# locuslab/icnn

Hardware: NVIDIA H100
Metric: inner-loop solves/sec (batch x iters) (higher is better)
Workload: dtype f32 (K1 PICNN f/grad) + f64 (K2 bundle solve)

## Files before the change

icnn_b200/csrc/bundle_pc.cu:

```cuda
#include "bundle_pc_kernel.cuh"

#include <cstdio>
#include <cstdlib>

namespace icnn {

#define ICNN_PC_DECL(NAME) cudaError_t launch_pc_##NAME(const PcArgs& a, const PcConfig& c, int B, cudaStream_t st)
ICNN_PC_DECL(1x1); ICNN_PC_DECL(1x2);
ICNN_PC_DECL(1x1_scalar); ICNN_PC_DECL(1x2_scalar);
ICNN_PC_DECL(8x2);
ICNN_PC_DECL(16x2); ICNN_PC_DECL(16x4);
ICNN_PC_DECL(v3_8x4);

ICNN_PC_DECL(1x1) { return launch_pc<1, 1, true>(a, c, B, st); }
ICNN_PC_DECL(1x2) { return launch_pc<1, 2, true>(a, c, B, st); }
ICNN_PC_DECL(1x1_scalar) { return launch_pc<1, 1, false>(a, c, B, st); }
ICNN_PC_DECL(1x2_scalar) { return launch_pc<1, 2, false>(a, c, B, st); }

struct PcTestEnv { bool v3, split5, seed, twolog; int pfa, pfb; };
static PcTestEnv pc_test_env() {
  PcTestEnv e = {true, false, true, false, 1, 8};
  if (const char* v = getenv("ICNN_PC_V3")) e.v3 = v[0] != '0';
  if (const char* v = getenv("ICNN_PC_LEGACY")) e.split5 = v[0] == '1';
  if (const char* v = getenv("ICNN_PC_SEED")) e.seed = v[0] != '0';
  if (const char* v = getenv("ICNN_PC_TWOLOG")) e.twolog = v[0] == '1';
  if (const char* v = getenv("ICNN_PC_PREFETCH")) {
    int pa = 0, pb = 0;
    if (sscanf(v, "%d,%d", &pa, &pb) == 2 && pa >= 0 && pa <= 8 && pb >= 0 && pb <= 64) { e.pfa = pa; e.pfb = pb; }
  }
  return e;
}

static bool pc_fits(int n, int KS, int wps, int nch, bool v3, PcConfig* out) {
  if (n > 128 * wps * nch) return false;
  PcConfig c;
  c.wps = wps; c.nch = nch; c.v3 = v3;
  c.npad = (n + 15) & ~15;
  c.vec = (n & 3) == 0;
  if (!c.vec && wps > 1) return false;
  c.smem = sizeof(double) * pc_group_doubles(c.npad, KS, wps, v3);
  if (c.smem > 227 * 1024) return false;
  if (v3) {
    if (!c.vec || 2 * (c.smem + 1024) > 228 * 1024) return false;
    c.minb = 2;
  } else if (wps == 16) c.minb = 1;
  else if (wps == 1) c.minb = 2;
  else
    c.minb = (c.smem + 1024) * (24 / wps) <= 228 * 1024 ? 3 : 2;
  *out = c;
  return true;
}

bool pick_pc(int n, int KS, PcConfig* out) {
  const bool allow_v3 = pc_test_env().v3;
  if (KS > 62) return false;
  if (n <= 128) return pc_fits(n, KS, 1, 1, false, out);
  if (n <= 256) return pc_fits(n, KS, 1, 2, false, out);
  if (n <= 1024) return false;
  if (n <= 2048) return pc_fits(n, KS, 8, 2, false, out);
  if (n <= 4096) return (allow_v3 && pc_fits(n, KS, 8, 4, true, out)) || pc_fits(n, KS, 16, 2, false, out);
  return pc_fits(n, KS, 16, 4, false, out);
}

int bundle_pc_launch(const icnn_bundle_cfg* cfg, const icnn_bundle_bufs* b, int t, const PcConfig& c, cudaStream_t st) {
  const PcTestEnv env = pc_test_env();
  PcArgs a;
  a.b = *b; a.c = *cfg; a.t = t; a.npad = c.npad;
  a.split5 = env.split5; a.seed = env.seed; a.twolog = env.twolog; a.pfa = env.pfa; a.pfb = env.pfb;
  cudaError_t e;
  if (c.v3) e = launch_pc_v3_8x4(a, c, b->B, st);
  else if (c.wps == 16) e = c.nch == 2 ? launch_pc_16x2(a, c, b->B, st) : launch_pc_16x4(a, c, b->B, st);
  else if (c.wps == 8) e = launch_pc_8x2(a, c, b->B, st);
  else if (c.vec) e = c.nch == 1 ? launch_pc_1x1(a, c, b->B, st) : launch_pc_1x2(a, c, b->B, st);
  else e = c.nch == 1 ? launch_pc_1x1_scalar(a, c, b->B, st) : launch_pc_1x2_scalar(a, c, b->B, st);
  if (e != cudaSuccess) {
    set_error("bundle_pc launch (wps=%d nch=%d v3=%d smem=%zu): %s", c.wps, c.nch, (int)c.v3, c.smem, cudaGetErrorString(e));
    return ICNN_E_CUDA;
  }
  return ICNN_OK;
}

}
```

icnn_b200/csrc/bundle_pc_kernel.cuh:

```cuda
#pragma once
#include "bundle_step_kernel.cuh"

namespace icnn {

struct PcArgs {
  icnn_bundle_bufs b;
  icnn_bundle_cfg c;
  int t;
  int npad;
  int pfa;
  int pfb;
  bool split5;
  bool seed;
  bool twolog;
#ifdef ICNN_PC_PHASES
  unsigned long long* ph;
#endif
};

enum PcPhase {
  PC_PH_APPEND = 0,
  PC_PH_SEED,
  PC_PH_U0,
  PC_PH_SWEEPA,
  PC_PH_KXK,
  PC_PH_SWEEPB,
  PC_PH_SIGMA,
  PC_PH_DIR2,
  PC_PH_UPDATE,
  PC_PH_COMMIT,
  PC_NPH
};
constexpr int PC_PH_SLOTS = 32;
#ifdef ICNN_PC_PHASES
#define PC_PHASE_START() long long pc_ph_t = clock64()
#define PC_PHASE(i)                                                                                              \
  do {                                                                                                           \
    if (threadIdx.x == 0) {                                                                                      \
      const long long pc_c = clock64();                                                                          \
      atomicAdd(A.ph + ((size_t)A.t * PC_NPH + (i)) * PC_PH_SLOTS + (blockIdx.x & (PC_PH_SLOTS - 1)),            \
                (unsigned long long)(pc_c - pc_ph_t));                                                           \
      pc_ph_t = pc_c;                                                                                            \
    }                                                                                                            \
  } while (0)
#else
#define PC_PHASE_START() do {} while (0)
#define PC_PHASE(i) do {} while (0)
#endif

__device__ __forceinline__ void prefetch_l2(const void* p) { asm volatile("prefetch.global.L2 [%0];" ::"l"(p)); }

constexpr int PC_NKV = 18;
constexpr int PC_NKV_V3 = 12;

__host__ __device__ inline size_t pc_group_doubles(int npad, int KS, int wps, bool v3) {
  size_t d = (size_t)(v3 ? 3 : 4) * npad + (size_t)KS * (KS + 1) / 2 +
             (size_t)(v3 ? PC_NKV_V3 : PC_NKV) * KS + KS  +
             8 * wps  + 16  + 4 ;
  return (d + 1) & ~(size_t)1;
}

__device__ __forceinline__ int lidx(int r, int c) { return r * (r + 1) / 2 + c; }

__device__ __forceinline__ double chol_dot(const double* a, const double* b, int c) {
  double t0 = 0.0, t1 = 0.0, t2 = 0.0, t3 = 0.0;
  int p = 0;
  for (; p + 3 < c; p += 4) {
    t0 = fma(a[p], b[p], t0);
    t1 = fma(a[p + 1], b[p + 1], t1);
    t2 = fma(a[p + 2], b[p + 2], t2);
    t3 = fma(a[p + 3], b[p + 3], t3);
  }
  for (; p < c; ++p) t0 = fma(a[p], b[p], t0);
  return (t0 + t1) + (t2 + t3);
}
template <bool K32>
__device__ __forceinline__ bool warp_cholesky_impl(double* L, double* invd, int k, int lane) {
  bool ok = true;
  const int r0 = lane, r1 = lane + 32;
  const int o0 = lidx(r0, 0), o1 = lidx(r1, 0);
  for (int c = 0; c < k; ++c) {
    const int oc = lidx(c, 0);
    double s0 = 0.0, s1 = 0.0;
    if (r0 >= c && r0 < k) s0 = L[o0 + c] - chol_dot(L + o0, L + oc, c);
    if (!K32) { if (r1 >= c && r1 < k) s1 = L[o1 + c] - chol_dot(L + o1, L + oc, c); }
    const double piv = K32 ? __shfl_sync(0xffffffffu, s0, c) : __shfl_sync(0xffffffffu, (c < 32) ? s0 : s1, c & 31);
    if (!(piv > 0.0) || !isfinite(piv)) { ok = false; break; }
    const double inv = rsqrt(piv);
    if (r0 > c && r0 < k) L[o0 + c] = s0 * inv;
    if (!K32) { if (r1 > c && r1 < k) L[o1 + c] = s1 * inv; }
    if (lane == 0) { L[oc + c] = piv * inv; invd[c] = inv; }
    __syncwarp();
  }
  __syncwarp();
  return ok;
}
__device__ inline bool warp_cholesky_p(double* L, double* invd, int k, int lane) {
  return k <= 32 ? warp_cholesky_impl<true>(L, invd, k, lane) : warp_cholesky_impl<false>(L, invd, k, lane);
}

template <int NR, bool K32>
__device__ __forceinline__ void warp_chol_fwd_impl(const double* L, const double* invd, int k, double (&b0)[NR],
                                                   double (&b1)[NR], int lane) {
  const int r0 = lane, r1 = lane + 32;
  const int o0 = lidx(r0, 0), o1 = lidx(r1, 0);
  for (int i = 0; i < k; ++i) {
    const double di = invd[i];
    const double l0 = (r0 > i && r0 < k) ? L[o0 + i] : 0.0;
    const double l1 = (!K32 && r1 > i && r1 < k) ? L[o1 + i] : 0.0;
#pragma unroll
    for (int q = 0; q < NR; ++q) {
      const double xi = (K32 ? __shfl_sync(0xffffffffu, b0[q], i) : __shfl_sync(0xffffffffu, (i < 32) ? b0[q] : b1[q], i & 31)) * di;
      b0[q] = (r0 == i) ? xi : fma(-l0, xi, b0[q]);
      if (!K32) b1[q] = (r1 == i) ? xi : fma(-l1, xi, b1[q]);
    }
  }
}
template <int NR, bool K32>
__device__ __forceinline__ void warp_chol_bwd_impl(const double* L, const double* invd, int k, double (&b0)[NR],
                                                   double (&b1)[NR], int lane) {
  const int r0 = lane, r1 = lane + 32;
  for (int i = k - 1; i >= 0; --i) {
    const double di = invd[i];
    const int oi = lidx(i, 0);
    const double l0 = (r0 < i) ? L[oi + r0] : 0.0;
    const double l1 = (!K32 && r1 < i) ? L[oi + r1] : 0.0;
#pragma unroll
    for (int q = 0; q < NR; ++q) {
      const double xi = (K32 ? __shfl_sync(0xffffffffu, b0[q], i) : __shfl_sync(0xffffffffu, (i < 32) ? b0[q] : b1[q], i & 31)) * di;
      b0[q] = (r0 == i) ? xi : fma(-l0, xi, b0[q]);
      if (!K32) b1[q] = (r1 == i) ? xi : fma(-l1, xi, b1[q]);
    }
  }
}
template <int NR, bool K32>
__device__ __forceinline__ void warp_chol_solve_impl(const double* L, const double* invd, int k, double (&b0)[NR],
                                                     double (&b1)[NR], int lane) {
  warp_chol_fwd_impl<NR, K32>(L, invd, k, b0, b1, lane);
  warp_chol_bwd_impl<NR, K32>(L, invd, k, b0, b1, lane);
}
template <int NR>
__device__ inline void warp_chol_solve_p(const double* L, const double* invd, int k, double (&b0)[NR],
                                         double (&b1)[NR], int lane) {
  if (k <= 32) warp_chol_solve_impl<NR, true>(L, invd, k, b0, b1, lane);
  else warp_chol_solve_impl<NR, false>(L, invd, k, b0, b1, lane);
}
template <bool K32>
__device__ __forceinline__ double warp_chol_solve_fwdsq_impl(const double* L, const double* invd, int k, double (&b0)[1],
                                                             double (&b1)[1], int lane) {
  warp_chol_fwd_impl<1, K32>(L, invd, k, b0, b1, lane);
  const double f0 = lane < k ? b0[0] : 0.0, f1 = (!K32 && lane + 32 < k) ? b1[0] : 0.0;
  const double fs = Grp<1>::wsum(fma(f0, f0, f1 * f1));
  warp_chol_bwd_impl<1, K32>(L, invd, k, b0, b1, lane);
  return fs;
}
__device__ inline double warp_chol_solve_fwdsq_p(const double* L, const double* invd, int k, double (&b0)[1],
                                                 double (&b1)[1], int lane) {
  return k <= 32 ? warp_chol_solve_fwdsq_impl<true>(L, invd, k, b0, b1, lane)
                 : warp_chol_solve_fwdsq_impl<false>(L, invd, k, b0, b1, lane);
}

__device__ __forceinline__ double step2(double v0, double d0, bool ok0, double v1, double d1, bool ok1) {
  double a = 1e300;
  bool any = false;
  if (ok0 && d0 < 0.0) { a = -v0 / d0; any = true; }
  if (ok1 && d1 < 0.0) { a = fmin(a, -v1 / d1); any = true; }
  a = Grp<1>::wmin(a);
  any = __any_sync(0xffffffffu, any);
  return any ? a : 1.0;
}

template <int WPS>
struct PcRed {
  double* red;
  int par;
  template <class G>
  __device__ __forceinline__ double sum(const G& g, double v) {
    v = Grp<WPS>::wsum(v);
    if (WPS == 1) { __syncwarp(); return v; }
    double* r = red + par * 4 * WPS;
    par ^= 1;
    if (g.lane == 0) r[g.warp] = v;
    g.sync();
    double a = 0.0;
#pragma unroll
    for (int w = 0; w < WPS; ++w) a += r[w];
    return a;
  }
  template <class G>
  __device__ __forceinline__ void min2(const G& g, double& a, double& b) {
    a = Grp<WPS>::wmin(a);
    b = Grp<WPS>::wmin(b);
    if (WPS == 1) { __syncwarp(); return; }
    double* r = red + par * 4 * WPS;
    par ^= 1;
    if (g.lane == 0) { r[g.warp] = a; r[WPS + g.warp] = b; }
    g.sync();
    double ra = r[0], rb = r[WPS];
#pragma unroll
    for (int w = 1; w < WPS; ++w) { ra = fmin(ra, r[w]); rb = fmin(rb, r[WPS + w]); }
    a = ra; b = rb;
  }
};

__device__ __forceinline__ double dweight(double y) { return fma(-y, y, y); }

template <int T, bool IL>
__device__ __forceinline__ int pc_tc(int cb, int npad) { return IL ? ::min(T, (npad - cb) >> 2) : 1; }
template <int T, bool IL>
__device__ __forceinline__ int pc_pos(int e, int npad) {
  if (!IL) return e;
  const int cb = e & ~(4 * T - 1);
  return cb + (e & 3) * pc_tc<T, IL>(cb, npad) + ((e - cb) >> 2);
}

template <int WPS, int NA, int NB, bool TRI, bool PSEUDO, bool VEC, bool IL, class G>
__device__ __forceinline__ void gram_sweep_pc(const G& g, const float* const* rowp, int k, int n, const double* yv,
                                              const double* rv, double* Lp, double* qk, double* wk, double* scratch,
                                              int scap, int a0, int b0, int pfd = 0) {
  constexpr int NT = TRI ? NA * (NA + 1) / 2 : NA * NB;
  constexpr int NL = TRI ? NB : NA + NB;
  double acc[NT][2];
#pragma unroll
  for (int t = 0; t < NT; ++t) acc[t][0] = acc[t][1] = 0.0;
  const int r = g.lane >> 2, q = g.lane & 3;
  const float* rp[NL];
  bool rok[NL];
#pragma unroll
  for (int b = 0; b < NL; ++b) {
    const int blk = TRI ? (b0 + b) : (b < NA ? a0 + b : b0 + (b - NA));
    const int row = blk * 8 + r - 2;
    rok[b] = row >= 0 && row < k;
    rp[b] = rowp[rok[b] ? row : 0] + 4 * q;
  }
  const bool ps = PSEUDO && r < 2;
  const double* yq = yv + 4 * q;
  const double* rq = rv + 4 * q;
  const int ngrp = (n + 15) >> 4;
  constexpr int NG = (NT <= 6) ? 2 : 1;
#pragma unroll 1
  for (int gi = g.warp; gi < ngrp; gi += NG * WPS) {
    float4 v[NG][NL];
#pragma unroll
    for (int u = 0; u < NG; ++u) {
      const int gu = gi + u * WPS;
      const int off = gu * 16;
      const int col = off + 4 * q;
      const bool gv = (u == 0) || gu < ngrp;
#pragma unroll
      for (int b = 0; b < NL; ++b) {
        v[u][b] = make_float4(0.f, 0.f, 0.f, 0.f);
        if (VEC) {
          if (gv && rok[b] && col < n) v[u][b] = *reinterpret_cast<const float4*>(rp[b] + off);
        } else if (gv && rok[b]) {
          const float* p = rp[b] + off;
          if (col < n) v[u][b].x = p[0];
          if (col + 1 < n) v[u][b].y = p[1];
          if (col + 2 < n) v[u][b].z = p[2];
          if (col + 3 < n) v[u][b].w = p[3];
        }
      }
    }
    if (pfd > 0) {
#pragma unroll
      for (int u = 0; u < NG; ++u) {
        const int col = (gi + (pfd * NG + u) * WPS) * 16 + 4 * q;
        if (col < n) {
#pragma unroll
          for (int b = 0; b < NL; ++b) if (rok[b]) prefetch_l2(rp[b] + (col - 4 * q));
        }
      }
    }
#pragma unroll
    for (int u = 0; u < NG; ++u) {
      const int gu = gi + u * WPS;
      if (u > 0 && gu >= ngrp) break;
      const int off = gu * 16;
      double ys[4];
      int p0 = 0, tc = 0;
      if (IL) {
        const int e0 = off + 4 * q, cb = e0 & ~(4 * 32 * WPS - 1);
        tc = pc_tc<32 * WPS, true>(cb, scap);
        p0 = cb + ((e0 - cb) >> 2);
#pragma unroll
        for (int s = 0; s < 4; ++s) ys[s] = yv[p0 + s * tc];
      } else {
        const double2 ya = *reinterpret_cast<const double2*>(yq + off);
        const double2 yb = *reinterpret_cast<const double2*>(yq + off + 2);
        ys[0] = ya.x; ys[1] = ya.y; ys[2] = yb.x; ys[3] = yb.y;
      }
      double dd[4] = {dweight(ys[0]), dweight(ys[1]), dweight(ys[2]), dweight(ys[3])};
      double pa[4] = {0.0, 0.0, 0.0, 0.0};
      if (PSEUDO && ps) {
        if (r == 0) {
          double rs[4];
          if (IL) {
#pragma unroll
            for (int s = 0; s < 4; ++s) rs[s] = rv[p0 + s * tc];
          } else {
            const double2 ra = *reinterpret_cast<const double2*>(rq + off);
            const double2 rb = *reinterpret_cast<const double2*>(rq + off + 2);
            rs[0] = ra.x; rs[1] = ra.y; rs[2] = rb.x; rs[3] = rb.y;
          }
#pragma unroll
          for (int s = 0; s < 4; ++s) pa[s] = dd[s] * rs[s];
        } else {
#pragma unroll
          for (int s = 0; s < 4; ++s) pa[s] = ys[s];
        }
      }
#pragma unroll
      for (int s = 0; s < 4; ++s) {
// ... 5 lines not shown
#pragma unroll
        for (int i = 0; i < NA; ++i) {
          const double af = (PSEUDO && i == 0) ? fma(f[0], dd[s], pa[s]) : f[i] * dd[s];
#pragma unroll
          for (int j = TRI ? i : 0; j < NB; ++j) { dmma884(acc[t][0], acc[t][1], af, f[TRI ? j : NA + j]); ++t; }
        }
      }
    }
  }
  if (WPS > 1) {
    constexpr int SLAB = NT * 64;
    const int cap = scap / SLAB;
    g.sync();
    if (cap >= 1) {
      int active = WPS;
      while (active > 1) {
        const int m = ::min(cap, active >> 1);
        if (g.warp >= active - m && g.warp < active) {
          double* sl = scratch + (size_t)(g.warp - (active - m)) * SLAB + g.lane;
#pragma unroll
          for (int t = 0; t < NT; ++t) { sl[(2 * t) * 32] = acc[t][0]; sl[(2 * t + 1) * 32] = acc[t][1]; }
        }
        g.sync();
        if (g.warp >= active - 2 * m && g.warp < active - m) {
          const double* sl = scratch + (size_t)(g.warp - (active - 2 * m)) * SLAB + g.lane;
#pragma unroll
          for (int t = 0; t < NT; ++t) { acc[t][0] += sl[(2 * t) * 32]; acc[t][1] += sl[(2 * t + 1) * 32]; }
        }
        active -= m;
        if (active > 1) g.sync();
      }
    } else {
      for (int wi = 1; wi < WPS; ++wi) {
        if (g.warp == wi) {
          int t = 0;
#pragma unroll
          for (int i = 0; i < NA; ++i)
#pragma unroll
            for (int j = TRI ? i : 0; j < NB; ++j) {
#pragma unroll
              for (int h = 0; h < 2; ++h) {
                const int ii = (a0 + i) * 8 + r, jj = (b0 + j) * 8 + 2 * q + h;
                if (jj >= 2 && jj < k + 2) {
                  if (ii < 2) { if (PSEUDO && i == 0) { double* d = (ii == 0 ? qk : wk) + (jj - 2); *d = (wi == 1 ? 0.0 : *d) + acc[t][h]; } }
                  else if (ii < k + 2 && (!(TRI && i == j) || jj >= ii)) { double* d = Lp + lidx(jj - 2, ii - 2); *d = (wi == 1 ? 0.0 : *d) + acc[t][h]; }
                }
              }
              ++t;
            }
        }
        g.sync();
      }
    }
  }
  if (g.warp == 0) {
    const bool addin = (WPS > 1) && (scap / (NT * 64) < 1);
    int t = 0;
#pragma unroll
    for (int i = 0; i < NA; ++i)
#pragma unroll
      for (int j = TRI ? i : 0; j < NB; ++j) {
#pragma unroll
        for (int h = 0; h < 2; ++h) {
          const int ii = (a0 + i) * 8 + r, jj = (b0 + j) * 8 + 2 * q + h;
          if (jj >= 2 && jj < k + 2) {
            if (ii < 2) {
              if (PSEUDO && i == 0) { double* d = (ii == 0 ? qk : wk) + (jj - 2); *d = (addin ? *d : 0.0) + acc[t][h]; }
            } else if (ii < k + 2 && (!(TRI && i == j) || jj >= ii)) {
              double* d = Lp + lidx(jj - 2, ii - 2);
              *d = (addin ? *d : 0.0) + acc[t][h];
            }
          }
        }
        ++t;
      }
    __syncwarp();
  }
}

template <int WPS, int NB, bool VEC, bool IL, class G>
__device__ __forceinline__ void gram_rect_pair_pc(const G& g, const float* const* rowp, int k, int n, const double* yv,
                                                  const double* rv, double* Lp, double* qk, double* wk, double* sx, int scap,
                                                  int pfd) {
  gram_sweep_pc<WPS, 2, NB, false, true, VEC, IL>(g, rowp, k, n, yv, rv, Lp, qk, wk, sx, scap, 0, 4, pfd);
  gram_sweep_pc<WPS, 2, NB, false, false, VEC, IL>(g, rowp, k, n, yv, rv, Lp, qk, wk, sx, scap, 2, 4, pfd);
}

template <int WPS, bool VEC, bool ONE5, bool IL, class G>
__device__ __forceinline__ void gram_pass_pc(const G& g, const float* const* rowp, int k, int n, const double* yv,
                                             const double* rv, double* Lp, double* qk, double* wk, double* sx, int scap,
                                             bool split5, int pfd) {
  const int rb = (k + 2 + 7) >> 3;
  if (rb == 1) gram_sweep_pc<WPS, 1, 1, true, true, VEC, IL>(g, rowp, k, n, yv, rv, Lp, qk, wk, sx, scap, 0, 0, pfd);
  else if (rb == 2) gram_sweep_pc<WPS, 2, 2, true, true, VEC, IL>(g, rowp, k, n, yv, rv, Lp, qk, wk, sx, scap, 0, 0, pfd);
  else if (rb == 3) gram_sweep_pc<WPS, 3, 3, true, true, VEC, IL>(g, rowp, k, n, yv, rv, Lp, qk, wk, sx, scap, 0, 0, pfd);
  else if (ONE5 && rb == 5 && !split5) {
    if constexpr (ONE5) gram_sweep_pc<WPS, 5, 5, true, true, VEC, IL>(g, rowp, k, n, yv, rv, Lp, qk, wk, sx, scap, 0, 0, pfd);
  } else {
    gram_sweep_pc<WPS, 4, 4, true, true, VEC, IL>(g, rowp, k, n, yv, rv, Lp, qk, wk, sx, scap, 0, 0, pfd);
    if (rb > 4) {
      const int r2 = rb - 4;
      if (r2 == 1) { gram_sweep_pc<WPS, 1, 1, true, false, VEC, IL>(g, rowp, k, n, yv, rv, Lp, qk, wk, sx, scap, 4, 4, pfd); gram_rect_pair_pc<WPS, 1, VEC, IL>(g, rowp, k, n, yv, rv, Lp, qk, wk, sx, scap, pfd); }
      else if (r2 == 2) { gram_sweep_pc<WPS, 2, 2, true, false, VEC, IL>(g, rowp, k, n, yv, rv, Lp, qk, wk, sx, scap, 4, 4, pfd); gram_rect_pair_pc<WPS, 2, VEC, IL>(g, rowp, k, n, yv, rv, Lp, qk, wk, sx, scap, pfd); }
      else if (r2 == 3) { gram_sweep_pc<WPS, 3, 3, true, false, VEC, IL>(g, rowp, k, n, yv, rv, Lp, qk, wk, sx, scap, 4, 4, pfd); gram_rect_pair_pc<WPS, 3, VEC, IL>(g, rowp, k, n, yv, rv, Lp, qk, wk, sx, scap, pfd); }
      else { gram_sweep_pc<WPS, 4, 4, true, false, VEC, IL>(g, rowp, k, n, yv, rv, Lp, qk, wk, sx, scap, 4, 4, pfd); gram_rect_pair_pc<WPS, 4, VEC, IL>(g, rowp, k, n, yv, rv, Lp, qk, wk, sx, scap, pfd); }
    }
  }
}

template <int T, bool VEC>
__device__ __forceinline__ int pc_col(int cb, int tid, int c) { return VEC ? cb + 4 * tid + c : cb + tid + c * T; }

template <int T, int NR, bool VEC, int UNR = 4>
__device__ __forceinline__ void col_dots_pc(const float* const* rowp, int k, int n, int cb, int tid,
                                            const double* const (&w)[NR], double (&acc)[NR][4], int pfr = 0) {
#pragma unroll
  for (int q = 0; q < NR; ++q)
#pragma unroll
    for (int c = 0; c < 4; ++c) acc[q][c] = 0.0;
  const bool in0 = VEC ? (cb + 4 * tid < n) : (cb + tid < n);
  const bool full = VEC ? in0 : (cb + tid + 3 * T < n);
#pragma unroll UNR
  for (int j = 0; j < k; ++j) {
    const float* p = rowp[j];
    float v[4] = {0.f, 0.f, 0.f, 0.f};
    if (VEC && pfr > 0 && in0) {
      const int jp = j + pfr;
      if (jp < k) prefetch_l2(rowp[jp] + cb + 4 * tid);
      else if (jp - k < k && cb + 4 * T + 4 * tid < n) prefetch_l2(rowp[jp - k] + cb + 4 * T + 4 * tid);
    }
    if (VEC) {
      if (in0) { const float4 x = *reinterpret_cast<const float4*>(p + cb + 4 * tid); v[0] = x.x; v[1] = x.y; v[2] = x.z; v[3] = x.w; }
    } else {
#pragma unroll
      for (int c = 0; c < 4; ++c) if (full || cb + tid + c * T < n) v[c] = p[cb + tid + c * T];
    }
#pragma unroll
    for (int q = 0; q < NR; ++q) {
      const double wq = w[q][j];
#pragma unroll
      for (int c = 0; c < 4; ++c) acc[q][c] = fma((double)v[c], wq, acc[q][c]);
    }
  }
}

__device__ __forceinline__ void ratio_min(double& nm, double& dn, double a, double b) {
  if (a * dn < nm * b) { nm = a; dn = b; }
}

struct PcKxk {
  double* Lp; double* invd; const double* zc; const double* scur; const double* wk; const double* hk; const double* qk;
  double* dza; double* dzp; double* dzq; double* dsa; double* sc; int* isc;
};
template <bool K32>
__device__ __forceinline__ void pc_kxk_stage(const PcKxk& io, int k, int lane, double pr) {
  double* Lp = io.Lp;
  const int j0 = lane, j1 = lane + 32;
  const bool v0 = j0 < k, v1ok = !K32 && j1 < k;
  const double tt = io.sc[0];
  const double z0 = v0 ? io.zc[j0] : 0.0, z1 = v1ok ? io.zc[j1] : 0.0;
  const double s0 = v0 ? io.scur[j0] : 0.0, s1 = v1ok ? io.scur[j1] : 0.0;
  const double rd0 = v0 ? ((io.wk[j0] + io.hk[j0]) - tt) + s0 : 0.0;
  const double rd1 = v1ok ? ((io.wk[j1] + io.hk[j1]) - tt) + s1 : 0.0;
  const double zs = Grp<1>::wsum(z0 + z1);
  const double dr = Grp<1>::wsum(fma(rd0, rd0, rd1 * rd1));
  const double rt = 1.0 - zs;
  const bool conv = (sqrt(pr + rt * rt) < 1e-8 && sqrt(dr) < 1e-8);
  if (conv) {
    if (lane == 0) io.isc[2] = 1;
  } else {
    if (v0) Lp[lidx(j0, j0)] += s0 / z0;
    if (v1ok) Lp[lidx(j1, j1)] += s1 / z1;
    __syncwarp();
    const bool ok = warp_cholesky_impl<K32>(Lp, io.invd, k, lane);
    if (!ok) { if (lane == 0) io.isc[3] = 1; }
    else {
      const double mu = Grp<1>::wsum(fma(s0, z0, s1 * z1)) / k;
      const double ra0 = v0 ? rd0 - io.qk[j0] - s0 : 0.0, ra1 = v1ok ? rd1 - io.qk[j1] - s1 : 0.0;
      const double rp0 = v0 ? mu / z0 : 0.0, rp1 = v1ok ? mu / z1 : 0.0;
      double b0[3] = {v0 ? 1.0 : 0.0, ra0, rp0}, b1[3] = {v1ok ? 1.0 : 0.0, ra1, rp1};
      warp_chol_solve_impl<3, K32>(Lp, io.invd, k, b0, b1, lane);
      const double w1s = Grp<1>::wsum(b0[0] + b1[0]);
      const double dta = (Grp<1>::wsum(fma(ra0, b0[0], ra1 * b1[0])) - rt) / w1s;
      const double dtp = Grp<1>::wsum(fma(rp0, b0[0], rp1 * b1[0])) / w1s;
      const double da0 = fma(-dta, b0[0], b0[1]), da1 = fma(-dta, b1[0], b1[1]);
      const double dp0 = fma(-dtp, b0[0], b0[2]), dp1 = fma(-dtp, b1[0], b1[2]);
      const double dsa0 = v0 ? -(s0 / z0) * (z0 + da0) : 0.0, dsa1 = v1ok ? -(s1 / z1) * (z1 + da1) : 0.0;
      const double rq0 = v0 ? -(dsa0 * da0) / z0 : 0.0, rq1 = v1ok ? -(dsa1 * da1) / z1 : 0.0;
      double c0[1] = {rq0}, c1[1] = {rq1};
      warp_chol_solve_impl<1, K32>(Lp, io.invd, k, c0, c1, lane);
      const double dtq = Grp<1>::wsum(fma(rq0, b0[0], rq1 * b1[0])) / w1s;
      if (v0) { io.dza[j0] = da0; io.dzp[j0] = dp0; io.dzq[j0] = fma(-dtq, b0[0], c0[0]); io.dsa[j0] = dsa0; }
      if (v1ok) { io.dza[j1] = da1; io.dzp[j1] = dp1; io.dzq[j1] = fma(-dtq, b1[0], c1[0]); io.dsa[j1] = dsa1; }
      if (lane == 0) { io.sc[1] = dta; io.sc[2] = dtp; io.sc[3] = dtq; }
    }
  }
  __syncwarp();
}

template <int WPS, int NCH, bool R80, bool VEC, bool V3>
__global__ void __launch_bounds__(WPS * 32, WPS == 16 ? 1 : (R80 ? 24 : 16) / WPS) bundle_pc_kernel(PcArgs A) {
  const icnn_bundle_bufs& b = A.b;
  const icnn_bundle_cfg& cf = A.c;
  if (b.nactive[A.t] == 0) return;
  extern __shared__ __align__(16) double smem_d[];
  constexpr int GPB = 1;
  constexpr int T = WPS * 32;
  static_assert(NCH == 1 || NCH == 2 || NCH == 4, "NCH");
  Grp<WPS> g;
  g.tid = threadIdx.x % T;
  g.lane = threadIdx.x & 31;
  g.warp = g.tid >> 5;
  g.gid = threadIdx.x / T;
  const int u = blockIdx.x * GPB + g.gid;
  if (u >= b.B) return;
  if (b.finished[u]) return;

  PC_PHASE_START();
  const int n = b.n, KS = b.KS, npad = A.npad;
  constexpr bool IL = V3;
  static_assert(!IL || VEC, "IL");
  double* base = smem_d + (size_t)g.gid * pc_group_doubles(npad, KS, WPS, V3);
  double* yv = base;
  double* uv = V3 ? nullptr : yv + npad;
  double* rv = V3 ? yv + npad : uv + npad;
  double* xv = rv + npad;
  double* Lp = xv + npad;
  double* kv = Lp + (size_t)KS * (KS + 1) / 2;
#define PCKV(i) (kv + (i) * KS)
  double* hk = PCKV(0);
  double* wk = PCKV(5);
  double* qk = PCKV(6);
  double* dza = PCKV(7);
  double* dzp = PCKV(8);
  double* dzq = PCKV(9);
  double* dsa = PCKV(10);
  double* invd = PCKV(11);
  double* tk = PCKV(V3 ? 7 : 12);
  double* ek = PCKV(V3 ? 8 : 13);
  double* rk = PCKV(V3 ? 9 : 14);
  const float** rowp = reinterpret_cast<const float**>(kv + (size_t)(V3 ? PC_NKV_V3 : PC_NKV) * KS);
  PcRed<WPS> red;
  red.red = reinterpret_cast<double*>(rowp + KS);
  red.par = 0;
  g.red = red.red;
  double* sc = red.red + 8 * WPS;
  int* isc = reinterpret_cast<int*>(sc + 16);

  const int k0 = b.count[u];
  const int k = k0 + 1;
  const int* permu = b.perm + (size_t)u * KS;
  float* Gu = b.G + (size_t)u * KS * n;
  double* hu = b.h + (size_t)u * KS;
  double* lamu = b.lam + (size_t)u * KS;
  double* rsu = b.rsum + (size_t)u * KS;
  double* gramu = b.gram + (size_t)u * KS * KS;
  double* yu = b.y + (size_t)u * n;
  const int slot_new = permu[k0];

  for (int j = g.tid; j < k; j += T) rowp[j] = Gu + (size_t)permu[j] * n;
  if (g.tid == 0) {
#pragma unroll
    for (int i = 0; i < 8; ++i) isc[i] = 0;
  }
  g.sync();
  const float* gnew = rowp[k0];

  {
    double hs = 0.0, rs = 0.0, bad = 0.0, ent = 0.0;
    double* ysrow = b.ys ? b.ys + ((size_t)u * KS + slot_new) * n : nullptr;
    for (int e = g.tid; e < n; e += T) {
      const double ge = (double)gnew[e];
      const double ye = yu[e];
      hs = fma(ge, ye, hs);
      rs += ge;
      if (!isfinite(ge)) bad = 1.0;
      if (ysrow) __stcs(ysrow + e, ye);
      if (b.iter_stats) ent += neg_entropy(ye);
    }
    if (b.iter_stats) ent = g.sum(ent);
    hs = g.sum(hs);
    rs = g.sum(rs);
    bad = g.max(bad);
    const double fu = b.f64 ? b.f64[u] : (double)b.f[u];
    if (g.tid == 0) { stat_add(b.iter_stats, A.t, 0, 1.0); stat_add(b.iter_stats, A.t, 6, fu + ent); }
    if (bad > 0.0 || !isfinite(fu)) {
      if (g.tid == 0) { b.status[u] = ICNN_ST_NONFINITE; b.finished[u] = 1; b.nIters[u] = A.t - 1; stat_add(b.iter_stats, A.t, 5, 1.0); }
      PC_PHASE(PC_PH_APPEND);
      return;
    }
    for (int j = g.warp; j < k; j += WPS) {
      const float* rj = rowp[j];
      double acc = 0.0;
      int diff = 0;
      for (int e = g.lane; e < n; e += 32) {
        const float a = rj[e], c = gnew[e];
        acc = fma((double)a, (double)c, acc);
        diff |= (a != c);
      }
      acc = Grp<WPS>::wsum(acc);
      diff = __any_sync(0xffffffffu, diff);
      if (g.lane == 0) { tk[j] = acc; ek[j] = diff ? 1.0 : 0.0; }
    }
    if (g.tid == 0) { hu[slot_new] = fu - hs; rsu[slot_new] = rs; sc[10] = fu - hs; sc[11] = rs; }
    g.sync();
    if (g.tid == 0) {
      int dup = 0;
      for (int j = 0; j < k0; ++j) dup |= (ek[j] == 0.0);
      isc[0] = dup;
    }
    g.sync();
  }
  bool dependent = false;
  if (k > n) dependent = true;
  else if (k0 > 0) {
    if (g.warp == 0) {
      for (int i = g.lane; i < k0; i += 32)
        for (int j = 0; j <= i; ++j) Lp[lidx(i, j)] = gramu[(size_t)permu[i] * KS + permu[j]];
      __syncwarp();
      const bool ok = warp_cholesky_p(Lp, invd, k0, g.lane);
      double fs = 0.0;
      if (ok) {
        double b0[1] = {g.lane < k0 ? tk[g.lane] : 0.0}, b1[1] = {g.lane + 32 < k0 ? tk[g.lane + 32] : 0.0};
        fs = warp_chol_solve_fwdsq_p(Lp, invd, k0, b0, b1, g.lane);
        if (g.lane < k0) rk[g.lane] = b0[0];
        if (g.lane + 32 < k0) rk[g.lane + 32] = b1[0];
      }
      double md = tk[k0];
      for (int j = g.lane; j < k0; j += 32) md = fmax(md, gramu[(size_t)permu[j] * KS + permu[j]]);
      md = Grp<1>::wmax(md);
      const bool clear = A.seed && ok && tk[k0] - fs > 100.0 * fmax(cf.rank_tol * cf.rank_tol * md, 1e-8 * md);
      if (g.lane == 0) { isc[1] = ok ? 1 : 0; isc[4] = clear ? 1 : 0; sc[9] = md; }
      __syncwarp();
    }
    g.sync();
    const double maxdiag = sc[9];
    if (isc[0]) dependent = true;
    else if (!isc[1] || isc[4]) dependent = false;
    else {
      const double thr2 = cf.rank_tol * cf.rank_tol * maxdiag;
      for (int rep = 0; rep < 2; ++rep) {
        double p = 0.0;
        col_pass<T>(rowp, k0, n, g.tid, rk, [&](int e, double a) {
          const double r = (rep ? xv[e] : (double)gnew[e]) - a;
          xv[e] = r;
          p = fma(r, r, p);
        });
        p = g.sum(p);
        if (p <= thr2) { dependent = true; break; }
        if (rep == 1 || p > 1e-8 * maxdiag) break;
        g.sync();
        for (int j = g.warp; j < k0; j += WPS) {
          double acc = 0.0;
          for (int e = g.lane; e < n; e += 32) acc = fma((double)rowp[j][e], xv[e], acc);
          acc = Grp<WPS>::wsum(acc);
          if (g.lane == 0) rk[j] = acc;
        }
        g.sync();
        if (g.warp == 0) {
          double b0[1] = {g.lane < k0 ? rk[g.lane] : 0.0}, b1[1] = {g.lane + 32 < k0 ? rk[g.lane + 32] : 0.0};
          warp_chol_solve_p<1>(Lp, invd, k0, b0, b1, g.lane);
          if (g.lane < k0) rk[g.lane] = b0[0];
          if (g.lane + 32 < k0) rk[g.lane + 32] = b1[0];
        }
        g.sync();
      }
    }
  } else {
    dependent = !(tk[0] > 0.0);
  }
  if (dependent) {
    if (g.tid == 0) { b.status[u] = ICNN_ST_RANK_STOP; b.finished[u] = 1; b.nIters[u] = A.t - 1; stat_add(b.iter_stats, A.t, 5, 1.0); }
    PC_PHASE(PC_PH_APPEND);
    return;
  }
  for (int j = g.tid; j < k; j += T) {
    gramu[(size_t)slot_new * KS + permu[j]] = tk[j];
    gramu[(size_t)permu[j] * KS + slot_new] = tk[j];
    hk[j] = (j == k0) ? sc[10] : hu[permu[j]];
    PCKV(1)[j] = 1.0 / k;
    PCKV(3)[j] = 1.0;
  }
  if (g.tid == 0) sc[0] = 1.0;
  for (int e = g.tid; e < npad; e += T) { yv[e] = 0.5; if (e >= n) rv[pc_pos<T, IL>(e, npad)] = 0.0; }
  g.sync();
  PC_PHASE(PC_PH_APPEND);

  const int maxit = cf.max_inner > 0 ? cf.max_inner : 20;
  int inner_its = 0, fail = 0;
  int zsel = 0;
  const int j0 = g.lane, j1 = g.lane + 32;
  const bool v0 = j0 < k, v1ok = j1 < k;
  bool seed0 = false;
  if (A.seed) {
    for (int p = g.tid; p < k * k; p += T) {
      const int i = p / k, j = p - i * k;
      if (j <= i) Lp[lidx(i, j)] = 0.25 * gramu[(size_t)permu[i] * KS + permu[j]];
    }
    g.sync();
    for (int i = g.tid; i < k; i += T) {
      const double* z = PCKV(1);
      double q = 0.0;
      for (int j = 0; j < k; ++j) q = fma(j <= i ? Lp[lidx(i, j)] : Lp[lidx(j, i)], z[j], q);
      qk[i] = q;
      wk[i] = 0.5 * rsu[permu[i]];
    }
    g.sync();
    const double rd0 = v0 ? ((wk[j0] + hk[j0]) - sc[0]) + PCKV(3)[j0] : 0.0;
    const double rd1 = v1ok ? ((wk[j1] + hk[j1]) - sc[0]) + PCKV(3)[j1] : 0.0;
    const double dr = Grp<1>::wsum(fma(rd0, rd0, rd1 * rd1));
    seed0 = sqrt(dr) >= 1e-6;
  }
  PC_PHASE(PC_PH_SEED);
  double pr = 0.0;
  {
    const double* const w1r[1] = {PCKV(1)};
#pragma unroll 1
    for (int ch = 0; ch < NCH; ++ch) {
      const int cb = ch * 4 * T;
      if (cb >= n) break;
      const int tc = pc_tc<T, IL>(cb, npad);
      double acc[1][4];
      col_dots_pc<T, 1, VEC>(rowp, k, n, cb, g.tid, w1r, acc);
#pragma unroll
      for (int c = 0; c < 4; ++c) {
        const int e = pc_col<T, VEC>(cb, g.tid, c);
        const int pe = IL ? cb + c * tc + g.tid : e;
        if (e < n) { if (!V3) uv[pe] = acc[0][c]; rv[pe] = acc[0][c]; pr = fma(acc[0][c], acc[0][c], pr); }
      }
    }
  }
  pr = red.sum(g, pr);
  PC_PHASE(PC_PH_U0);
#pragma unroll 1
  for (int it = 0; it < maxit; ++it) {
    double* zc = PCKV(1 + zsel);
    double* scur = PCKV(3 + zsel);
    const bool seeded = seed0 && it == 0;
    if (!seeded) gram_pass_pc<WPS, VEC, V3, IL>(g, rowp, k, n, yv, rv, Lp, qk, wk, xv, npad, A.split5, V3 ? A.pfa : 0);
    PC_PHASE(PC_PH_SWEEPA);
    if (g.warp == 0) {
      const PcKxk io{Lp, invd, zc, scur, wk, hk, qk, dza, dzp, dzq, dsa, sc, isc};
      if (k <= 32) pc_kxk_stage<true>(io, k, g.lane, pr);
      else pc_kxk_stage<false>(io, k, g.lane, pr);
    }
    g.sync();
    PC_PHASE(PC_PH_KXK);
    if (isc[2]) break;
    if (isc[3]) { fail = 1; break; }
    inner_its = it + 1;
    double x2a[4], x2b[4], x2c[4], x2d[4];
    double n1 = 1.0, d1 = 0.0, n2 = 1.0, d2 = 0.0;
    {
      const double* const w3[3] = {dza, dzp, dzq};
#pragma unroll 1
      for (int ch = 0; ch < NCH; ++ch) {
        const int cb = ch * 4 * T;
        if (cb >= n) break;
        const int tc = pc_tc<T, IL>(cb, npad);
        double acc[3][4];
        col_dots_pc<T, 3, VEC, V3 ? 8 : 4>(rowp, k, n, cb, g.tid, w3, acc, V3 ? A.pfb : 0);
#pragma unroll
        for (int c = 0; c < 4; ++c) {
          const int e = pc_col<T, VEC>(cb, g.tid, c);
          const int pe = IL ? cb + c * tc + g.tid : e;
          if (e < n) {
            const double ye = yv[pe];
            const double dy = -dweight(ye) * (rv[pe] + acc[0][c]);
            if (dy < 0.0) ratio_min(n1, d1, ye, -dy);
            if (dy > 0.0) ratio_min(n2, d2, 1.0 - ye, dy);
            xv[pe] = acc[0][c] + acc[2][c];
          }
          const double v2 = acc[1][c];
          if (ch == 0) x2a[c] = v2; else if (ch == 1) x2b[c] = v2; else if (ch == 2) x2c[c] = v2; else x2d[c] = v2;
        }
      }
    }
    double st = d1 > 0.0 ? n1 / d1 : 1e300, st2 = d2 > 0.0 ? n2 / d2 : 1e300;
    red.min2(g, st, st2);
    st = fmin(st > 1e299 ? 1.0 : st, st2 > 1e299 ? 1.0 : st2);
    PC_PHASE(PC_PH_SWEEPB);
    const double z0 = v0 ? zc[j0] : 0.0, z1 = v1ok ? zc[j1] : 0.0;
    const double s0 = v0 ? scur[j0] : 0.0, s1 = v1ok ? scur[j1] : 0.0;
    const double da0 = v0 ? dza[j0] : 0.0, da1 = v1ok ? dza[j1] : 0.0;
    const double dsa0 = v0 ? dsa[j0] : 0.0, dsa1 = v1ok ? dsa[j1] : 0.0;
    double dz0, dz1, ds0, ds1, dtt, sig;
    {
      const double alpha = fmin(fmin(step2(z0, da0, v0, z1, da1, v1ok), step2(s0, dsa0, v0, s1, dsa1, v1ok)), fmin(st, 1.0));
      const double num = Grp<1>::wsum(fma(s0 + alpha * dsa0, z0 + alpha * da0, (s1 + alpha * dsa1) * (z1 + alpha * da1)));
      const double den = Grp<1>::wsum(fma(s0, z0, s1 * z1));
      const double sg = num / den;
      sig = sg * sg * sg;
      const double mu = den / k;
      const double dzc0 = v0 ? fma(sig, dzp[j0], dzq[j0]) : 0.0, dzc1 = v1ok ? fma(sig, dzp[j1], dzq[j1]) : 0.0;
      const double rc0 = v0 ? -(mu * sig - dsa0 * da0) / s0 : 0.0, rc1 = v1ok ? -(mu * sig - dsa1 * da1) / s1 : 0.0;
      dz0 = da0 + dzc0; dz1 = da1 + dzc1;
      ds0 = v0 ? dsa0 - (s0 / z0) * (rc0 + dzc0) : 0.0;
      ds1 = v1ok ? dsa1 - (s1 / z1) * (rc1 + dzc1) : 0.0;
      dtt = sc[1] + fma(sig, sc[2], sc[3]);
    }
    PC_PHASE(PC_PH_SIGMA);
    n1 = 1.0; d1 = 0.0; n2 = 1.0; d2 = 0.0;
#pragma unroll 1
    for (int ch = 0; ch < NCH; ++ch) {
      const int cb = ch * 4 * T;
      if (cb >= n) break;
      const int tc = pc_tc<T, IL>(cb, npad);
#pragma unroll
      for (int c = 0; c < 4; ++c) {
        const int e = pc_col<T, VEC>(cb, g.tid, c);
        const int pe = IL ? cb + c * tc + g.tid : e;
        const double v2 = (ch == 0) ? x2a[c] : (ch == 1) ? x2b[c] : (ch == 2) ? x2c[c] : x2d[c];
        if (e < n) {
          const double ye = yv[pe];
          const double du = fma(sig, v2, xv[pe]);
          const double dy = -dweight(ye) * (rv[pe] + du);
          if (dy < 0.0) ratio_min(n1, d1, ye, -dy);
          if (dy > 0.0) ratio_min(n2, d2, 1.0 - ye, dy);
          if (V3) xv[pe] = du;
          else { xv[pe] = dy; rv[pe] = du; }
        }
      }
    }
    st = d1 > 0.0 ? n1 / d1 : 1e300; st2 = d2 > 0.0 ? n2 / d2 : 1e300;
    red.min2(g, st, st2);
    st = fmin(st > 1e299 ? 1.0 : st, st2 > 1e299 ? 1.0 : st2);
    double a = fmin(fmin(step2(s0, ds0, v0, s1, ds1, v1ok), step2(z0, dz0, v0, z1, dz1, v1ok)), st);
    a = fmax(0.0, fmin(1.0, 0.99 * a));
    if (g.warp == 0) {
      double* zn = PCKV(2 - zsel);
      double* snew = PCKV(4 - zsel);
      if (v0) { zn[j0] = fma(a, dz0, z0); snew[j0] = fma(a, ds0, s0); }
      if (v1ok) { zn[j1] = fma(a, dz1, z1); snew[j1] = fma(a, ds1, s1); }
      if (g.lane == 0) sc[0] += a * dtt;
    }
    zsel ^= 1;
    PC_PHASE(PC_PH_DIR2);
    pr = 0.0;
#pragma unroll 1
    for (int ch = 0; ch < NCH; ++ch) {
      const int cb = ch * 4 * T;
      if (cb >= n) break;
      const int tc = pc_tc<T, IL>(cb, npad);
#pragma unroll (WPS == 1 ? 1 : 4)
      for (int c = 0; c < 4; ++c) {
        const int e = pc_col<T, VEC>(cb, g.tid, c);
        const int pe = IL ? cb + c * tc + g.tid : e;
        if (e < n) {
          if (V3) {
            const double yo = yv[pe], ro = rv[pe], du = xv[pe];
            const double dy = -dweight(yo) * (ro + du);
            const double ye = fma(a, dy, yo);
            double r;
            if (A.twolog) {
              const double uo = ro - log(yo / (1.0 - yo));
              r = log(ye / (1.0 - ye)) + fma(a, du, uo);
            } else {
              r = fma(a, du, ro) + log((ye * (1.0 - yo)) / (yo * (1.0 - ye)));
            }
            yv[pe] = ye; rv[pe] = r;
            pr = fma(r, r, pr);
          } else {
            const double ye = fma(a, xv[pe], yv[pe]);
            const double ue = fma(a, rv[pe], uv[pe]);
            const double r = log(ye / (1.0 - ye)) + ue;
            yv[pe] = ye; uv[pe] = ue; rv[pe] = r;
            pr = fma(r, r, pr);
          }
        }
      }
    }
    pr = red.sum(g, pr);
    PC_PHASE(PC_PH_UPDATE);
  }
  g.sync();
  const double* zfin = PCKV(1 + zsel);

  double bad = 0.0;
  for (int e = g.tid; e < n; e += T) {
    const double ye = yv[pc_pos<T, IL>(e, npad)];
    if (!isfinite(ye)) bad = 1.0;
    yu[e] = ye;
    b.y32[(size_t)u * n + e] = (float)ye;
  }
  bad = g.max(bad);
  if (g.tid == 0) {
    int nk = 0, nd = 0;
    int* oldp = reinterpret_cast<int*>(tk);
    int* dropped = oldp + KS;
    int* pw = b.perm + (size_t)u * KS;
    for (int j = 0; j < k; ++j) oldp[j] = pw[j];
    for (int j = 0; j < k; ++j) {
      const double lj = zfin[j];
      if (lj > cf.prune_thr) { pw[nk++] = oldp[j]; lamu[oldp[j]] = lj; }
      else dropped[nd++] = oldp[j];
    }
    for (int j = 0; j < nd; ++j) pw[nk + j] = dropped[j];
    b.count[u] = nk;
    int fin = 0;
    int stt = ICNN_ST_RUNNING;
// ... 36 lines not shown
```

Measured before the change: 206,800.

## Factor the KxK Cholesky across the whole CTA instead of one warp

Adds a block-wide right-looking Cholesky that spreads the packed lower-triangular elements over all threads of a multi-warp group. It is used for the seed factorization and the per-iteration KxK factor when k is at least 14, with an env switch to fall back to the single-warp path. The aim is to stop the other warps idling while warp 0 factors serially. The cost is one block sync per column and extra barriers, and the phase-timing macros are refactored into a struct.

```diff
diff --git a/icnn_b200/csrc/bundle_pc.cu b/icnn_b200/csrc/bundle_pc.cu
--- a/icnn_b200/csrc/bundle_pc.cu
+++ b/icnn_b200/csrc/bundle_pc.cu
@@ -2,6 +2,7 @@
 
 #include <cstdio>
 #include <cstdlib>
+#include <cstring>
 
 namespace icnn {
 
@@ -17,13 +18,14 @@
 ICNN_PC_DECL(1x1_scalar) { return launch_pc<1, 1, false>(a, c, B, st); }
 ICNN_PC_DECL(1x2_scalar) { return launch_pc<1, 2, false>(a, c, B, st); }
 
-struct PcTestEnv { bool v3, split5, seed, twolog; int pfa, pfb; };
+struct PcTestEnv { bool v3, split5, seed, twolog, kxkwarp; int pfa, pfb; };
 static PcTestEnv pc_test_env() {
-  PcTestEnv e = {true, false, true, false, 1, 8};
+  PcTestEnv e = {true, false, true, false, false, 1, 8};
   if (const char* v = getenv("ICNN_PC_V3")) e.v3 = v[0] != '0';
   if (const char* v = getenv("ICNN_PC_LEGACY")) e.split5 = v[0] == '1';
   if (const char* v = getenv("ICNN_PC_SEED")) e.seed = v[0] != '0';
   if (const char* v = getenv("ICNN_PC_TWOLOG")) e.twolog = v[0] == '1';
+  if (const char* v = getenv("ICNN_PC_KXK")) e.kxkwarp = strcmp(v, "warp") == 0;
   if (const char* v = getenv("ICNN_PC_PREFETCH")) {
     int pa = 0, pb = 0;
     if (sscanf(v, "%d,%d", &pa, &pb) == 2 && pa >= 0 && pa <= 8 && pb >= 0 && pb <= 64) { e.pfa = pa; e.pfb = pb; }
@@ -66,7 +68,7 @@
   const PcTestEnv env = pc_test_env();
   PcArgs a;
   a.b = *b; a.c = *cfg; a.t = t; a.npad = c.npad;
-  a.split5 = env.split5; a.seed = env.seed; a.twolog = env.twolog; a.pfa = env.pfa; a.pfb = env.pfb;
+  a.split5 = env.split5; a.seed = env.seed; a.twolog = env.twolog; a.kxkwarp = env.kxkwarp; a.pfa = env.pfa; a.pfb = env.pfb;
   cudaError_t e;
   if (c.v3) e = launch_pc_v3_8x4(a, c, b->B, st);
   else if (c.wps == 16) e = c.nch == 2 ? launch_pc_16x2(a, c, b->B, st) : launch_pc_16x4(a, c, b->B, st);
diff --git a/icnn_b200/csrc/bundle_pc_kernel.cuh b/icnn_b200/csrc/bundle_pc_kernel.cuh
--- a/icnn_b200/csrc/bundle_pc_kernel.cuh
+++ b/icnn_b200/csrc/bundle_pc_kernel.cuh
@@ -13,6 +13,7 @@
   bool split5;
   bool seed;
   bool twolog;
+  bool kxkwarp;
 #ifdef ICNN_PC_PHASES
   unsigned long long* ph;
 #endif
@@ -23,7 +24,9 @@
   PC_PH_SEED,
   PC_PH_U0,
   PC_PH_SWEEPA,
-  PC_PH_KXK,
+  PC_PH_CONV,
+  PC_PH_FACTOR,
+  PC_PH_SOLVES,
   PC_PH_SWEEPB,
   PC_PH_SIGMA,
   PC_PH_DIR2,
@@ -33,20 +36,30 @@
 };
 constexpr int PC_PH_SLOTS = 32;
 #ifdef ICNN_PC_PHASES
-#define PC_PHASE_START() long long pc_ph_t = clock64()
-#define PC_PHASE(i)                                                                                              \
-  do {                                                                                                           \
-    if (threadIdx.x == 0) {                                                                                      \
-      const long long pc_c = clock64();                                                                          \
-      atomicAdd(A.ph + ((size_t)A.t * PC_NPH + (i)) * PC_PH_SLOTS + (blockIdx.x & (PC_PH_SLOTS - 1)),            \
-                (unsigned long long)(pc_c - pc_ph_t));                                                           \
-      pc_ph_t = pc_c;                                                                                            \
-    }                                                                                                            \
-  } while (0)
+struct PcPh {
+  unsigned long long* ph;
+  int t;
+  long long last;
+  __device__ __forceinline__ void start(const PcArgs& A) { ph = A.ph; t = A.t; last = clock64(); }
+  __device__ __forceinline__ void mark(int i) {
+    if (threadIdx.x == 0) {
+      const long long c = clock64();
+      atomicAdd(ph + ((size_t)t * PC_NPH + i) * PC_PH_SLOTS + (blockIdx.x & (PC_PH_SLOTS - 1)),
+                (unsigned long long)(c - last));
+      last = c;
+    }
+  }
+};
 #else
-#define PC_PHASE_START() do {} while (0)
-#define PC_PHASE(i) do {} while (0)
+struct PcPh {
+  __device__ __forceinline__ void start(const PcArgs&) {}
+  __device__ __forceinline__ void mark(int) {}
+};
 #endif
+#define PC_PHASE_START() \
+  PcPh pc_ph;             \
+  pc_ph.start(A)
+#define PC_PHASE(i) pc_ph.mark(i)
 
 __device__ __forceinline__ void prefetch_l2(const void* p) { asm volatile("prefetch.global.L2 [%0];" ::"l"(p)); }
 
@@ -158,6 +171,62 @@
                                                  double (&b1)[1], int lane) {
   return k <= 32 ? warp_chol_solve_fwdsq_impl<true>(L, invd, k, b0, b1, lane)
                  : warp_chol_solve_fwdsq_impl<false>(L, invd, k, b0, b1, lane);
+}
+
+constexpr int PC_KXK_CTA_MIN = 14;
+template <int WPS, class G, class Init>
+__device__ __noinline__ bool cta_cholesky(const G& g, double* L, double* invd, int k, Init init) {
+  constexpr int T = 32 * WPS;
+  constexpr int NE = (62 * 63 / 2 + T - 1) / T;
+  const int nel = k * (k + 1) / 2;
+  int oi[NE];
+#pragma unroll
+  for (int m = 0; m < NE; ++m) {
+    const int p = g.tid + m * T;
+    oi[m] = 0;
+    if (p < nel) {
+      int i = (int)((sqrtf((float)(8 * p + 1)) - 1.f) * 0.5f);
+      if (lidx(i + 1, 0) <= p) ++i;
+      if (lidx(i, 0) > p) --i;
+      oi[m] = lidx(i, 0);
+      init(i, p - oi[m], L[p]);
+      if (p == 0) {
+        const double piv = L[0];
+        const bool ok = piv > 0.0 && isfinite(piv);
+        const double inv = ok ? rsqrt(piv) : 0.0;
+        if (ok) L[0] = piv * inv;
+        invd[0] = inv;
+      }
+    }
+  }
+  g.sync();
+  double invp = 0.0;
+  for (int c = 0; c < k; ++c) {
+    const double inv = invd[c];
+    if (!(inv > 0.0)) return false;
+    const int dnext = lidx(c + 1, c + 1);
+#pragma unroll
+    for (int m = 0; m < NE; ++m) {
+      const int p = g.tid + m * T, j = p - oi[m];
+      if (p >= nel) break;
+      if (j == c - 1) {
+        if (p != lidx(j, j)) L[p] *= invp;
+      } else if (j > c) {
+        const double v = L[p] - (L[oi[m] + c] * inv) * (L[lidx(j, c)] * inv);
+        if (p == dnext) {
+          const bool ok = v > 0.0 && isfinite(v);
+          const double iv = ok ? rsqrt(v) : 0.0;
+          L[p] = ok ? v * iv : v;
+          invd[c + 1] = iv;
+        } else {
+          L[p] = v;
+        }
+      }
+    }
+    invp = inv;
+    g.sync();
+  }
+  return true;
 }
 
 __device__ __forceinline__ double step2(double v0, double d0, bool ok0, double v1, double d1, bool ok1) {
@@ -469,50 +538,81 @@
   double* Lp; double* invd; const double* zc; const double* scur; const double* wk; const double* hk; const double* qk;
   double* dza; double* dzp; double* dzq; double* dsa; double* sc; int* isc;
 };
+struct PcKl { double z0, z1, s0, s1, rd0, rd1, rt; bool v0, v1; };
 template <bool K32>
-__device__ __forceinline__ void pc_kxk_stage(const PcKxk& io, int k, int lane, double pr) {
-  double* Lp = io.Lp;
+__device__ __forceinline__ bool pc_kxk_conv(const PcKxk& io, int k, int lane, double pr, PcKl& e) {
   const int j0 = lane, j1 = lane + 32;
-  const bool v0 = j0 < k, v1ok = !K32 && j1 < k;
+  e.v0 = j0 < k; e.v1 = !K32 && j1 < k;
   const double tt = io.sc[0];
-  const double z0 = v0 ? io.zc[j0] : 0.0, z1 = v1ok ? io.zc[j1] : 0.0;
-  const double s0 = v0 ? io.scur[j0] : 0.0, s1 = v1ok ? io.scur[j1] : 0.0;
-  const double rd0 = v0 ? ((io.wk[j0] + io.hk[j0]) - tt) + s0 : 0.0;
-  const double rd1 = v1ok ? ((io.wk[j1] + io.hk[j1]) - tt) + s1 : 0.0;
-  const double zs = Grp<1>::wsum(z0 + z1);
-  const double dr = Grp<1>::wsum(fma(rd0, rd0, rd1 * rd1));
-  const double rt = 1.0 - zs;
-  const bool conv = (sqrt(pr + rt * rt) < 1e-8 && sqrt(dr) < 1e-8);
-  if (conv) {
+  e.z0 = e.v0 ? io.zc[j0] : 0.0; e.z1 = e.v1 ? io.zc[j1] : 0.0;
+  e.s0 = e.v0 ? io.scur[j0] : 0.0; e.s1 = e.v1 ? io.scur[j1] : 0.0;
+  e.rd0 = e.v0 ? ((io.wk[j0] + io.hk[j0]) - tt) + e.s0 : 0.0;
+  e.rd1 = e.v1 ? ((io.wk[j1] + io.hk[j1]) - tt) + e.s1 : 0.0;
+  const double zs = Grp<1>::wsum(e.z0 + e.z1);
+  const double dr = Grp<1>::wsum(fma(e.rd0, e.rd0, e.rd1 * e.rd1));
+  e.rt = 1.0 - zs;
+  return sqrt(pr + e.rt * e.rt) < 1e-8 && sqrt(dr) < 1e-8;
+}
+template <bool K32>
+__device__ __forceinline__ void pc_kxk_solves(const PcKxk& io, int k, int lane, const PcKl& e) {
+  const int j0 = lane, j1 = lane + 32;
+  const bool v0 = e.v0, v1ok = e.v1;
+  const double z0 = e.z0, z1 = e.z1, s0 = e.s0, s1 = e.s1;
+  const double mu = Grp<1>::wsum(fma(s0, z0, s1 * z1)) / k;
+  const double ra0 = v0 ? e.rd0 - io.qk[j0] - s0 : 0.0, ra1 = v1ok ? e.rd1 - io.qk[j1] - s1 : 0.0;
+  const double rp0 = v0 ? mu / z0 : 0.0, rp1 = v1ok ? mu / z1 : 0.0;
+  double b0[3] = {v0 ? 1.0 : 0.0, ra0, rp0}, b1[3] = {v1ok ? 1.0 : 0.0, ra1, rp1};
+  warp_chol_solve_impl<3, K32>(io.Lp, io.invd, k, b0, b1, lane);
+  const double w1s = Grp<1>::wsum(b0[0] + b1[0]);
+  const double dta = (Grp<1>::wsum(fma(ra0, b0[0], ra1 * b1[0])) - e.rt) / w1s;
+  const double dtp = Grp<1>::wsum(fma(rp0, b0[0], rp1 * b1[0])) / w1s;
+  const double da0 = fma(-dta, b0[0], b0[1]), da1 = fma(-dta, b1[0], b1[1]);
+  const double dp0 = fma(-dtp, b0[0], b0[2]), dp1 = fma(-dtp, b1[0], b1[2]);
+  const double dsa0 = v0 ? -(s0 / z0) * (z0 + da0) : 0.0, dsa1 = v1ok ? -(s1 / z1) * (z1 + da1) : 0.0;
+  const double rq0 = v0 ? -(dsa0 * da0) / z0 : 0.0, rq1 = v1ok ? -(dsa1 * da1) / z1 : 0.0;
+  double c0[1] = {rq0}, c1[1] = {rq1};
+  warp_chol_solve_impl<1, K32>(io.Lp, io.invd, k, c0, c1, lane);
+  const double dtq = Grp<1>::wsum(fma(rq0, b0[0], rq1 * b1[0])) / w1s;
+  if (v0) { io.dza[j0] = da0; io.dzp[j0] = dp0; io.dzq[j0] = fma(-dtq, b0[0], c0[0]); io.dsa[j0] = dsa0; }
+  if (v1ok) { io.dza[j1] = da1; io.dzp[j1] = dp1; io.dzq[j1] = fma(-dtq, b1[0], c1[0]); io.dsa[j1] = dsa1; }
+  if (lane == 0) { io.sc[1] = dta; io.sc[2] = dtp; io.sc[3] = dtq; }
+}
+template <bool K32>
+__device__ __forceinline__ void pc_kxk_stage(const PcKxk& io, int k, int lane, double pr, PcPh& ph) {
+  PcKl e;
+  if (pc_kxk_conv<K32>(io, k, lane, pr, e)) {
     if (lane == 0) io.isc[2] = 1;
+    ph.mark(PC_PH_CONV);
   } else {
-    if (v0) Lp[lidx(j0, j0)] += s0 / z0;
-    if (v1ok) Lp[lidx(j1, j1)] += s1 / z1;
+    if (e.v0) io.Lp[lidx(lane, lane)] += e.s0 / e.z0;
+    if (e.v1) io.Lp[lidx(lane + 32, lane + 32)] += e.s1 / e.z1;
     __syncwarp();
-    const bool ok = warp_cholesky_impl<K32>(Lp, io.invd, k, lane);
+    ph.mark(PC_PH_CONV);
+    const bool ok = warp_cholesky_impl<K32>(io.Lp, io.invd, k, lane);
+    ph.mark(PC_PH_FACTOR);
     if (!ok) { if (lane == 0) io.isc[3] = 1; }
-    else {
-      const double mu = Grp<1>::wsum(fma(s0, z0, s1 * z1)) / k;
-      const double ra0 = v0 ? rd0 - io.qk[j0] - s0 : 0.0, ra1 = v1ok ? rd1 - io.qk[j1] - s1 : 0.0;
-      const double rp0 = v0 ? mu / z0 : 0.0, rp1 = v1ok ? mu / z1 : 0.0;
-      double b0[3] = {v0 ? 1.0 : 0.0, ra0, rp0}, b1[3] = {v1ok ? 1.0 : 0.0, ra1, rp1};
-      warp_chol_solve_impl<3, K32>(Lp, io.invd, k, b0, b1, lane);
-      const double w1s = Grp<1>::wsum(b0[0] + b1[0]);
-      const double dta = (Grp<1>::wsum(fma(ra0, b0[0], ra1 * b1[0])) - rt) / w1s;
-      const double dtp = Grp<1>::wsum(fma(rp0, b0[0], rp1 * b1[0])) / w1s;
-      const double da0 = fma(-dta, b0[0], b0[1]), da1 = fma(-dta, b1[0], b1[1]);
-      const double dp0 = fma(-dtp, b0[0], b0[2]), dp1 = fma(-dtp, b1[0], b1[2]);
-      const double dsa0 = v0 ? -(s0 / z0) * (z0 + da0) : 0.0, dsa1 = v1ok ? -(s1 / z1) * (z1 + da1) : 0.0;
-      const double rq0 = v0 ? -(dsa0 * da0) / z0 : 0.0, rq1 = v1ok ? -(dsa1 * da1) / z1 : 0.0;
-      double c0[1] = {rq0}, c1[1] = {rq1};
-      warp_chol_solve_impl<1, K32>(Lp, io.invd, k, c0, c1, lane);
-      const double dtq = Grp<1>::wsum(fma(rq0, b0[0], rq1 * b1[0])) / w1s;
-      if (v0) { io.dza[j0] = da0; io.dzp[j0] = dp0; io.dzq[j0] = fma(-dtq, b0[0], c0[0]); io.dsa[j0] = dsa0; }
-      if (v1ok) { io.dza[j1] = da1; io.dzp[j1] = dp1; io.dzq[j1] = fma(-dtq, b1[0], c1[0]); io.dsa[j1] = dsa1; }
-      if (lane == 0) { io.sc[1] = dta; io.sc[2] = dtp; io.sc[3] = dtq; }
-    }
+    else pc_kxk_solves<K32>(io, k, lane, e);
   }
   __syncwarp();
+}
+template <int WPS, bool K32, class G>
+__device__ __forceinline__ void pc_kxk_stage_cta(const G& g, const PcKxk& io, int k, double pr, PcPh& ph) {
+  PcKl e;
+  if (pc_kxk_conv<K32>(io, k, g.lane, pr, e)) {
+    if (g.tid == 0) io.isc[2] = 1;
+    ph.mark(PC_PH_CONV);
+    return;
+  }
+  ph.mark(PC_PH_CONV);
+  const double* zc = io.zc;
+  const double* scur = io.scur;
+  const bool ok = cta_cholesky<WPS>(g, io.Lp, io.invd, k, [&](int i, int j, double& v) { if (i == j) v += scur[j] / zc[j]; });
+  ph.mark(PC_PH_FACTOR);
+  if (g.warp == 0) {
+    if (!ok) { if (g.lane == 0) io.isc[3] = 1; }
+    else pc_kxk_solves<K32>(io, k, g.lane, e);
+    __syncwarp();
+  }
 }
 
 template <int WPS, int NCH, bool R80, bool VEC, bool V3>
@@ -631,11 +731,16 @@
   bool dependent = false;
   if (k > n) dependent = true;
   else if (k0 > 0) {
+    bool cta = false, ok = false;
+    if constexpr (WPS > 1) cta = !A.kxkwarp && k0 >= PC_KXK_CTA_MIN;
+    if (cta) ok = cta_cholesky<WPS>(g, Lp, invd, k0, [&](int i, int j, double& v) { v = gramu[(size_t)permu[i] * KS + permu[j]]; });
     if (g.warp == 0) {
-      for (int i = g.lane; i < k0; i += 32)
-        for (int j = 0; j <= i; ++j) Lp[lidx(i, j)] = gramu[(size_t)permu[i] * KS + permu[j]];
-      __syncwarp();
-      const bool ok = warp_cholesky_p(Lp, invd, k0, g.lane);
+      if (!cta) {
+        for (int i = g.lane; i < k0; i += 32)
+          for (int j = 0; j <= i; ++j) Lp[lidx(i, j)] = gramu[(size_t)permu[i] * KS + permu[j]];
+        __syncwarp();
+        ok = warp_cholesky_p(Lp, invd, k0, g.lane);
+      }
       double fs = 0.0;
       if (ok) {
         double b0[1] = {g.lane < k0 ? tk[g.lane] : 0.0}, b1[1] = {g.lane + 32 < k0 ? tk[g.lane + 32] : 0.0};
@@ -756,13 +861,21 @@
     const bool seeded = seed0 && it == 0;
     if (!seeded) gram_pass_pc<WPS, VEC, V3, IL>(g, rowp, k, n, yv, rv, Lp, qk, wk, xv, npad, A.split5, V3 ? A.pfa : 0);
     PC_PHASE(PC_PH_SWEEPA);
-    if (g.warp == 0) {
+    {
       const PcKxk io{Lp, invd, zc, scur, wk, hk, qk, dza, dzp, dzq, dsa, sc, isc};
-      if (k <= 32) pc_kxk_stage<true>(io, k, g.lane, pr);
-      else pc_kxk_stage<false>(io, k, g.lane, pr);
+      bool cta = false;
+      if constexpr (WPS > 1) cta = !A.kxkwarp && k >= PC_KXK_CTA_MIN;
+      if (cta) {
+        g.sync();
+        if (k <= 32) pc_kxk_stage_cta<WPS, true>(g, io, k, pr, pc_ph);
+        else pc_kxk_stage_cta<WPS, false>(g, io, k, pr, pc_ph);
+      } else if (g.warp == 0) {
+        if (k <= 32) pc_kxk_stage<true>(io, k, g.lane, pr, pc_ph);
+        else pc_kxk_stage<false>(io, k, g.lane, pr, pc_ph);
+      }
     }
     g.sync();
-    PC_PHASE(PC_PH_KXK);
+    PC_PHASE(PC_PH_SOLVES);
     if (isc[2]) break;
     if (isc[3]) { fail = 1; break; }
     inner_its = it + 1;
```

Result: faster. 212,000 (median of 6 runs) (+2.5%).
